# ranrhuang/SPFSplatV2

Hardware: AMD Instinct MI355X
Metric: Mpixels/s fwd+bwd, 256x256 @ ~65k Gaussians (higher is better)
Workload: dtype f32; 1 GPU; C2: 65536 pixel-aligned Gaussians/scene, 1 SH coefficient(s) per channel (sh_degree 0), 256x256, 8 scenes x 4 views per GPU per step, decoder fwd + MSE + bwd to all Gaussian parameters and poses; loss=spfsplatv2_amd.mse_loss (fused HIP), scenes_per_gpu=8, sh_coeffs=1, pair_buffer=planned from step 0 (x1.25 = 2814155 pairs), verified on device, launch=hip-graph replay, api=batched: one decoder call for all renders

## Files before the change

### spfsplatv2_amd/csrc/binning.hip

```cpp
#include <atomic>

#include "spf_common.h"
#include "launchers.h"

namespace spf {

uint32_t dense_threshold();
uint32_t dense_threshold_fwd();

constexpr int kScanThreads = 1024;

__global__ __launch_bounds__(kScanThreads) void spf_tile_scan_kernel(const uint32_t* __restrict__ count,
                                                                     uint32_t* __restrict__ start,
                                                                     uint32_t* __restrict__ fill,
                                                                     const uint32_t* __restrict__ flags,
                                                                     uint32_t dense_thr,
                                                                     uint32_t* __restrict__ counters, int n,
                                                                     const uint32_t* __restrict__ blk_total,
                                                                     uint32_t* __restrict__ blk_base, int nb) {
    constexpr int kWaves = kScanThreads / kWave;
    __shared__ uint32_t s_a[kWaves], s_b[kWaves], s_mx[kWaves], s_dn[kWaves];
    const int lane = threadIdx.x & (kWave - 1), wave = threadIdx.x >> 6;
    const int sega = ((n + kWaves - 1) / kWaves + kWave - 1) / kWave * kWave;
    const int segb = ((nb + kWaves - 1) / kWaves + kWave - 1) / kWave * kWave;
    const int a0 = min(n, wave * sega), a1 = min(n, a0 + sega), b0 = min(nb, wave * segb), b1 = min(nb, b0 + segb);
    uint32_t sa = 0, sb = 0, mx = 0, dn = 0;
    for (int i = a0 + lane; i < a1; i += kWave) {
        const uint32_t c = count[i];
        sa += c;
        mx = max(mx, c);
        dn += tile_is_dense(flags[i], c, dense_thr) ? 1u : 0u;
    }
    for (int i = b0 + lane; i < b1; i += kWave) sb += blk_total[i];
    sa = wave_sum_u32(sa); sb = wave_sum_u32(sb); mx = wave_max_u32(mx); dn = wave_sum_u32(dn);
    if (lane == 0) { s_a[wave] = sa; s_b[wave] = sb; s_mx[wave] = mx; s_dn[wave] = dn; }
    __syncthreads();
    uint32_t runa = 0, runb = 0, total = 0, gmax = 0, dense = 0;
#pragma unroll
    for (int w = 0; w < kWaves; ++w) {
        if (w < wave) { runa += s_a[w]; runb += s_b[w]; }
        total += s_a[w];
        gmax = max(gmax, s_mx[w]);
        dense += s_dn[w];
    }
    for (int i0 = a0; i0 < a1; i0 += kWave) {
        const int i = i0 + lane;
        const uint32_t c = i < a1 ? count[i] : 0u;
        const uint32_t inc = wave_iscan_u32(c);
        if (i < a1) { start[i] = runa + inc - c; fill[i] = 0u; }
        runa += (uint32_t)__builtin_amdgcn_readlane((int)inc, kWave - 1);
    }
    for (int i0 = b0; i0 < b1; i0 += kWave) {
        const int i = i0 + lane;
        const uint32_t c = i < b1 ? blk_total[i] : 0u;
        const uint32_t inc = wave_iscan_u32(c);
        if (i < b1) blk_base[i] = runb + inc - c;
        runb += (uint32_t)__builtin_amdgcn_readlane((int)inc, kWave - 1);
    }
    if (threadIdx.x == 0) {
        start[n] = total;
        counters[0] = total;
        counters[1] = gmax;
        counters[2] = 0;
        counters[3] = dense;
    }
}

__global__ __launch_bounds__(kScanThreads) void spf_tile_scan_render_kernel(const uint32_t* __restrict__ count,
                                                                            uint32_t* __restrict__ start,
                                                                            const uint32_t* __restrict__ flags,
                                                                            uint32_t dense_thr,
                                                                            uint32_t* __restrict__ counters, int T,
                                                                            const uint32_t* __restrict__ blk_total,
                                                                            uint32_t* __restrict__ blk_base, int nb) {
    constexpr int kWaves = kScanThreads / kWave;
    __shared__ uint32_t s_red[kWaves], s_a[kWaves], s_b[kWaves], s_mx[kWaves], s_dn[kWaves];
    const int r = blockIdx.x, R = gridDim.x;
    const int lane = threadIdx.x & (kWave - 1), wave = threadIdx.x >> 6;
    uint32_t pre = 0;
    for (int i = threadIdx.x; i < r * T; i += kScanThreads) pre += count[i];
    pre = wave_sum_u32(pre);
    if (lane == 0) s_red[wave] = pre;
    count += (size_t)r * T; flags += (size_t)r * T; start += (size_t)r * T;
    blk_total += (size_t)r * nb; blk_base += (size_t)r * nb;
    const int sega = ((T + kWaves - 1) / kWaves + kWave - 1) / kWave * kWave;
    const int segb = ((nb + kWaves - 1) / kWaves + kWave - 1) / kWave * kWave;
    const int a0 = min(T, wave * sega), a1 = min(T, a0 + sega), b0 = min(nb, wave * segb), b1 = min(nb, b0 + segb);
    uint32_t sa = 0, sb = 0, mx = 0, dn = 0;
    for (int i = a0 + lane; i < a1; i += kWave) {
        const uint32_t c = count[i];
        sa += c;
        mx = max(mx, c);
        dn += tile_is_dense(flags[i], c, dense_thr) ? 1u : 0u;
    }
    for (int i = b0 + lane; i < b1; i += kWave) sb += blk_total[i];
    sa = wave_sum_u32(sa); sb = wave_sum_u32(sb); mx = wave_max_u32(mx); dn = wave_sum_u32(dn);
    if (lane == 0) { s_a[wave] = sa; s_b[wave] = sb; s_mx[wave] = mx; s_dn[wave] = dn; }
    __syncthreads();
    uint32_t base = 0, runa = 0, runb = 0, total = 0, gmax = 0, dense = 0;
#pragma unroll
    for (int w = 0; w < kWaves; ++w) {
        base += s_red[w];
        if (w < wave) { runa += s_a[w]; runb += s_b[w]; }
        total += s_a[w];
        gmax = max(gmax, s_mx[w]);
        dense += s_dn[w];
    }
    runa += base; runb += base;
    for (int i0 = a0; i0 < a1; i0 += kWave) {
        const int i = i0 + lane;
        const uint32_t c = i < a1 ? count[i] : 0u;
        const uint32_t inc = wave_iscan_u32(c);
        if (i < a1) start[i] = runa + inc - c;
        runa += (uint32_t)__builtin_amdgcn_readlane((int)inc, kWave - 1);
    }
    for (int i0 = b0; i0 < b1; i0 += kWave) {
        const int i = i0 + lane;
        const uint32_t c = i < b1 ? blk_total[i] : 0u;
        const uint32_t inc = wave_iscan_u32(c);
        if (i < b1) blk_base[i] = runb + inc - c;
        runb += (uint32_t)__builtin_amdgcn_readlane((int)inc, kWave - 1);
    }
    if (threadIdx.x == 0) {
        if (gmax) atomicMax(&counters[1], gmax);
        if (dense) atomicAdd(&counters[3], dense);
        if (r == R - 1) {
            start[T] = base + total;
            counters[0] = base + total;
        }
    }
}

__global__ __launch_bounds__(kBlock) void spf_bin_pairs_kernel(const float* __restrict__ zkey,
                                                               const uint32_t* __restrict__ rect,
                                                               const uint32_t* __restrict__ tile_start,
                                                               uint32_t* __restrict__ tile_fill,
                                                               uint32_t* __restrict__ counters,
                                                               uint64_t* __restrict__ pairs, uint64_t capacity,
                                                               const uint32_t* __restrict__ blk_base,
                                                               uint32_t* __restrict__ pair_off,
                                                               int G, int T, int tiles_x, int lds,
                                                               uint32_t max_tile_hint) {
    extern __shared__ __attribute__((aligned(16))) uint32_t s_bin[];
    __shared__ uint32_t s_wtot[4];
    uint32_t* s_cnt = s_bin;
    uint32_t* s_base = s_bin + T;
    const int r = blockIdx.y;
    const int g = blockIdx.x * kBlock + threadIdx.x;
    if (r == 0 && g == 0) {
        uint32_t flag = counters[0] > capacity ? 1u : 0u;
        if (max_tile_hint != 0u && counters[1] > max_tile_hint) flag |= 2u;
        if (flag) counters[2] = flag;
    }
    if (counters[0] > capacity) return;
    const bool live = g < G;
    const size_t rg = (size_t)r * G + (live ? g : 0);
    const size_t tb = (size_t)r * T;
    const uint32_t rc = live ? rect[rg] : 0u;
    const float zk = live ? zkey[rg] : 0.f;
    const uint32_t bbase = blk_base[(size_t)r * gridDim.x + blockIdx.x];
    constexpr int kPre = 4;
    uint32_t ts_pre[kPre] = {0u, 0u, 0u, 0u};
    const bool pre = lds && T <= kPre * kBlock;
    if (pre) {
#pragma unroll
        for (int k = 0; k < kPre; ++k)
            if (threadIdx.x + k * kBlock < T) ts_pre[k] = tile_start[tb + threadIdx.x + k * kBlock];
    }
    const int x0 = rc & 0xff, y0 = (rc >> 8) & 0xff, x1 = (rc >> 16) & 0xff, y1 = rc >> 24;
    const bool any = x1 > x0 && y1 > y0;
    const int lane = threadIdx.x & 63, wave = threadIdx.x >> 6;
    const uint32_t cnt = any ? (uint32_t)((x1 - x0) * (y1 - y0)) : 0u;
    const uint32_t inc = wave_iscan_u32(cnt);
    if (lane == kWave - 1) s_wtot[wave] = inc;
    if (lds)
        for (int t = threadIdx.x; t < T; t += kBlock) s_cnt[t] = 0;
    __syncthreads();
    {
        uint32_t off = bbase + inc - cnt;
        for (int w = 0; w < wave; ++w) off += s_wtot[w];
        if (live) reinterpret_cast<uint2*>(pair_off)[rg] = make_uint2(rc, off);
    }
    const uint64_t key = any ? (((uint64_t)__float_as_uint(zk) << 32) | (uint32_t)g) : 0ull;
    if (!lds) {
        if (any)
            for (int ty = y0; ty < y1; ++ty)
                for (int tx = x0; tx < x1; ++tx) {
                    const size_t t = tb + ty * tiles_x + tx;
                    pairs[tile_start[t] + atomicAdd(&tile_fill[t], 1u)] = key;
                }
        return;
    }
    const bool single = any && cnt == 1u;
    const int stile = single ? y0 * tiles_x + x0 : -1;
    const LaneRun run = lane_runs(stile, lane);
    const bool run_head = single && run.head == lane;
    if (run_head) atomicAdd(&s_cnt[stile], (uint32_t)run.len);
    if (any && !single)
        for (int ty = y0; ty < y1; ++ty)
            for (int tx = x0; tx < x1; ++tx) atomicAdd(&s_cnt[ty * tiles_x + tx], 1u);
    __syncthreads();
    if (pre) {
#pragma unroll
        for (int k = 0; k < kPre; ++k) {
            const int t = threadIdx.x + k * kBlock;
            if (t < T) {
                const uint32_t c = s_cnt[t];
                if (c) {
                    s_base[t] = ts_pre[k] + atomicAdd(&tile_fill[tb + t], c);
                    s_cnt[t] = 0;
                }
            }
        }
    } else {
        for (int t = threadIdx.x; t < T; t += kBlock) {
            const uint32_t c = s_cnt[t];
            if (c) {
                s_base[t] = tile_start[tb + t] + atomicAdd(&tile_fill[tb + t], c);
                s_cnt[t] = 0;
            }
        }
    }
    __syncthreads();
    uint32_t first = 0u;
    if (run_head) first = atomicAdd(&s_cnt[stile], (uint32_t)run.len);
    first = (uint32_t)__shfl((int)first, run.head, kWave);
    if (single) pairs[s_base[stile] + first + (uint32_t)(lane - run.head)] = key;
    if (any && !single)
        for (int ty = y0; ty < y1; ++ty)
            for (int tx = x0; tx < x1; ++tx) {
                const int t = ty * tiles_x + tx;
                pairs[s_base[t] + atomicAdd(&s_cnt[t], 1u)] = key;
            }
}

template <int VB>
__global__ __launch_bounds__(kBlock) void spf_bin_pairs_views_kernel(const float* __restrict__ zkey,
                                                                     const uint32_t* __restrict__ rect,
                                                                     const uint32_t* __restrict__ tile_start,
                                                                     uint32_t* __restrict__ tile_fill,
                                                                     uint32_t* __restrict__ counters,
                                                                     uint64_t* __restrict__ pairs, uint64_t capacity,
                                                                     const uint32_t* __restrict__ blk_base,
                                                                     uint32_t* __restrict__ pair_off,
                                                                     int G, int T, int tiles_x, int V, int nvb,
                                                                     uint32_t max_tile_hint) {
    extern __shared__ __attribute__((aligned(16))) uint32_t s_bin[];
    __shared__ uint32_t s_wtot[VB][4];
    uint32_t* const s_cnt = s_bin;
    uint32_t* const s_base = s_bin + VB * T;
    const int sc = blockIdx.y / nvb, vb = blockIdx.y - sc * nvb;
    const int v0 = vb * VB, nv = min(VB, V - v0);
    const int r0 = sc * V + v0;
    const int g = blockIdx.x * kBlock + threadIdx.x;
    if (blockIdx.y == 0 && g == 0) {
        uint32_t flag = counters[0] > capacity ? 1u : 0u;
        if (max_tile_hint != 0u && counters[1] > max_tile_hint) flag |= 2u;
        if (flag) counters[2] = flag;
    }
    if (counters[0] > capacity) return;
    const bool live = g < G;
    const int lane = threadIdx.x & 63, wave = threadIdx.x >> 6;
    constexpr int kPre = 4;
    uint32_t rc[VB], bbase[VB], ts_pre[VB][kPre];
    float zk[VB];
#pragma unroll
    for (int k = 0; k < VB; ++k) {
        const bool on = k < nv;
        const size_t rg = (size_t)(r0 + (on ? k : 0)) * G + (live ? g : 0);
        rc[k] = (on && live) ? rect[rg] : 0u;
        zk[k] = (on && live) ? zkey[rg] : 0.f;
        bbase[k] = on ? blk_base[(size_t)(r0 + k) * gridDim.x + blockIdx.x] : 0u;
#pragma unroll
        for (int j = 0; j < kPre; ++j) {
            const int t = threadIdx.x + j * kBlock;
            ts_pre[k][j] = (on && t < T) ? tile_start[(size_t)(r0 + k) * T + t] : 0u;
        }
    }
    uint32_t cnt[VB], inc[VB];
#pragma unroll
    for (int k = 0; k < VB; ++k) {
        const int x0 = rc[k] & 0xff, y0 = (rc[k] >> 8) & 0xff, x1 = (rc[k] >> 16) & 0xff, y1 = rc[k] >> 24;
        cnt[k] = (x1 > x0 && y1 > y0) ? (uint32_t)((x1 - x0) * (y1 - y0)) : 0u;
        inc[k] = wave_iscan_u32(cnt[k]);
        if (lane == kWave - 1) s_wtot[k][wave] = inc[k];
    }
    for (int t = threadIdx.x; t < VB * T; t += kBlock) s_cnt[t] = 0;
    __syncthreads();
#pragma unroll
    for (int k = 0; k < VB; ++k) {
        uint32_t off = bbase[k] + inc[k] - cnt[k];
        for (int w = 0; w < wave; ++w) off += s_wtot[k][w];
        if (live && k < nv) reinterpret_cast<uint2*>(pair_off)[(size_t)(r0 + k) * G + g] = make_uint2(rc[k], off);
    }
    LaneRun run[VB];
    int stile[VB];
#pragma unroll
    for (int k = 0; k < VB; ++k) {
        const int x0 = rc[k] & 0xff, y0 = (rc[k] >> 8) & 0xff, x1 = (rc[k] >> 16) & 0xff, y1 = rc[k] >> 24;
        stile[k] = cnt[k] == 1u ? y0 * tiles_x + x0 : -1;
        run[k] = lane_runs(stile[k], lane);
        uint32_t* __restrict__ c = s_cnt + k * T;
        if (cnt[k] == 1u && run[k].head == lane) atomicAdd(&c[stile[k]], (uint32_t)run[k].len);
        if (cnt[k] > 1u)
            for (int ty = y0; ty < y1; ++ty)
                for (int tx = x0; tx < x1; ++tx) atomicAdd(&c[ty * tiles_x + tx], 1u);
    }
    __syncthreads();
#pragma unroll
    for (int k = 0; k < VB; ++k)
#pragma unroll
        for (int j = 0; j < kPre; ++j) {
            const int t = threadIdx.x + j * kBlock;
            if (k < nv && t < T) {
                const uint32_t c = s_cnt[k * T + t];
                if (c) {
                    s_base[k * T + t] = ts_pre[k][j] + atomicAdd(&tile_fill[(size_t)(r0 + k) * T + t], c);
                    s_cnt[k * T + t] = 0;
                }
            }
        }
    __syncthreads();
#pragma unroll
    for (int k = 0; k < VB; ++k) {
        const int x0 = rc[k] & 0xff, y0 = (rc[k] >> 8) & 0xff, x1 = (rc[k] >> 16) & 0xff, y1 = rc[k] >> 24;
        const uint64_t key = ((uint64_t)__float_as_uint(zk[k]) << 32) | (uint32_t)g;
        uint32_t* __restrict__ c = s_cnt + k * T;
        const uint32_t* __restrict__ bs = s_base + k * T;
        const bool single = cnt[k] == 1u;
        uint32_t first = 0u;
        if (single && run[k].head == lane) first = atomicAdd(&c[stile[k]], (uint32_t)run[k].len);
        first = (uint32_t)__shfl((int)first, run[k].head, kWave);
        if (single) pairs[bs[stile[k]] + first + (uint32_t)(lane - run[k].head)] = key;
        if (cnt[k] > 1u)
            for (int ty = y0; ty < y1; ++ty)
                for (int tx = x0; tx < x1; ++tx) {
                    const int t = ty * tiles_x + tx;
                    pairs[bs[t] + atomicAdd(&c[t], 1u)] = key;
                }
    }
}

constexpr int kOrderClasses = 64;
constexpr int kOrderWindow = 256;
static_assert(kOrderClasses == kWave, "the class bases are one wave's prefix sum");
__host__ __device__ inline int order_windows(int RT) { return ((RT >> 3) + kOrderWindow - 1) / kOrderWindow; }
__device__ __forceinline__ void tile_order_block(int id, const uint32_t* __restrict__ count,
                                                 const uint32_t* __restrict__ flags, uint2* __restrict__ order, int RT,
                                                 int T, uint32_t cap, uint32_t dense_thr, uint32_t dense_thr_fwd) {
    auto dense_bits = [&](uint32_t f, uint32_t n) {
        return (tile_is_dense(f, n, dense_thr) ? kOrderDenseBwd : 0u) | (tile_is_dense(f, n, dense_thr_fwd) ? kOrderDenseFwd : 0u);
    };
    __shared__ uint32_t s_cnt[kOrderClasses];
    const int nwin = order_windows(RT), x = id / nwin, w = id - x * nwin;
    const XcdMap xm = xcd_map(RT, T);
    const int per = RT >> 3, j0 = w * kOrderWindow, lo = x * per + j0, len = min(kOrderWindow, per - j0);
    const int nthr = (int)blockDim.x;
    if (w + 1 < nwin) {
        for (int i = threadIdx.x; i < len; i += nthr) {
            const int vid = xcd_tile(xm, T, x, j0 + i);
            const uint32_t n = min(count[vid], cap);
            order[lo + i] = make_uint2((uint32_t)vid | dense_bits(flags[vid], n), n);
        }
        return;
    }
    if (threadIdx.x < kOrderClasses) s_cnt[threadIdx.x] = 0u;
    __syncthreads();
    auto cls = [&](uint32_t n) {
        return (uint32_t)(kOrderClasses - 1) - min((uint32_t)(kOrderClasses - 1), n * (uint32_t)kOrderClasses / (cap + 1u));
    };
    for (int i = threadIdx.x; i < len; i += nthr) atomicAdd(&s_cnt[cls(min(count[xcd_tile(xm, T, x, j0 + i)], cap))], 1u);
    __syncthreads();
    uint32_t base = 0u;
    if (threadIdx.x < kWave) {
        const uint32_t c = s_cnt[threadIdx.x];
        base = wave_iscan_u32(c) - c;
    }
    __syncthreads();
    if (threadIdx.x < kWave) s_cnt[threadIdx.x] = base;
    __syncthreads();
    for (int i = threadIdx.x; i < len; i += nthr) {
        const int vid = xcd_tile(xm, T, x, j0 + i);
        const uint32_t n = min(count[vid], cap);
        const uint32_t pos = atomicAdd(&s_cnt[cls(n)], 1u);
        order[lo + pos] = make_uint2((uint32_t)vid | dense_bits(flags[vid], n), n);
    }
}
__global__ __launch_bounds__(kBlock) void spf_tile_order_kernel(const uint32_t* __restrict__ count,
                                                                const uint32_t* __restrict__ flags,
                                                                uint2* __restrict__ order, int RT, int T, uint32_t cap,
                                                                uint32_t dense_thr, uint32_t dense_thr_fwd) {
    tile_order_block((int)blockIdx.x, count, flags, order, RT, T, cap, dense_thr, dense_thr_fwd);
}

template <int THREADS>
__global__ __launch_bounds__(THREADS) void spf_sort_tiles_lds_kernel(TileLists tl,
                                                                     const uint32_t* __restrict__ counters,
                                                                     uint64_t* __restrict__ pairs,
                                                                     uint64_t capacity, uint32_t lo, uint32_t hi) {
    extern __shared__ __attribute__((aligned(16))) unsigned char smem_raw[];
    uint64_t* s = reinterpret_cast<uint64_t*>(smem_raw);
    if (counters[0] > capacity) return;
    uint32_t b, n;
    tile_range(tl, blockIdx.x, b, n);
    if (n <= lo || n > hi) return;
    uint64_t* __restrict__ p = pairs + b;
    for (uint32_t i = threadIdx.x; i < n; i += THREADS) s[i] = p[i];
    __syncthreads();
    uint32_t m = 1;
    while (m < n) m <<= 1;
    const uint32_t half = m >> 1;
    for (uint32_t k = 2; k <= m; k <<= 1) {
        for (uint32_t j = k >> 1; j > 0; j >>= 1) {
            const uint32_t mask = (j == (k >> 1)) ? (k - 1) : j;
            for (uint32_t i = threadIdx.x; i < half; i += THREADS) {
                const uint32_t a = ((i & ~(j - 1)) << 1) | (i & (j - 1));
                const uint32_t c = a ^ mask;
                if (c < n) {
                    const uint64_t x = s[a], y = s[c];
                    if (x > y) { s[a] = y; s[c] = x; }
                }
            }
            __syncthreads();
        }
    }
    for (uint32_t i = threadIdx.x; i < n; i += THREADS) p[i] = s[i];
}

__device__ __forceinline__ void cswap_u64(uint64_t& a, uint64_t& b) {
    const bool sw = a > b;
    const uint64_t lo = sw ? b : a, hi = sw ? a : b;
    a = lo;
    b = hi;
}

template <int CTRL>
__device__ __forceinline__ uint32_t dpp_mov_u32(uint32_t v) {
    return (uint32_t)__builtin_amdgcn_update_dpp((int)v, (int)v, CTRL, 0xf, 0xf, true);
}
template <int MASK>
__device__ __forceinline__ uint32_t lane_xor_u32(uint32_t v) {
    if constexpr (MASK == 1) return dpp_mov_u32<0xB1>(v);
    else if constexpr (MASK == 2) return dpp_mov_u32<0x4E>(v);
    else if constexpr (MASK == 3) return dpp_mov_u32<0x1B>(v);
    else if constexpr (MASK == 4) return dpp_mov_u32<0x1B>(dpp_mov_u32<0x141>(v));
    else if constexpr (MASK == 7) return dpp_mov_u32<0x141>(v);
    else if constexpr (MASK == 8) return dpp_mov_u32<0x128>(v);
    else if constexpr (MASK == 15) return dpp_mov_u32<0x140>(v);
    else return (uint32_t)__shfl_xor((int)v, MASK, kWave);
}
template <int MASK>
__device__ __forceinline__ uint64_t lane_xor_u64(uint64_t v) {
    return ((uint64_t)lane_xor_u32<MASK>((uint32_t)(v >> 32)) << 32) | lane_xor_u32<MASK>((uint32_t)v);
}

template <int E, int J>
__device__ __forceinline__ void thread_steps_down(uint64_t (&r)[E]) {
    if constexpr (J >= 1) {
#pragma unroll
        for (int s = 0; s < E; ++s)
            if (s < (s ^ J)) cswap_u64(r[s], r[s ^ J]);
        thread_steps_down<E, J / 2>(r);
    }
}
template <int E, int K>
__device__ __forceinline__ void merges_inside(uint64_t (&r)[E]) {
    if constexpr (K <= E) {
#pragma unroll
        for (int s = 0; s < E; ++s)
            if (s < (s ^ (K - 1))) cswap_u64(r[s], r[s ^ (K - 1)]);
        thread_steps_down<E, K / 4>(r);
        merges_inside<E, 2 * K>(r);
    }
}
template <int E, int MASK, bool MIRROR>
__device__ __forceinline__ void lane_step(uint64_t (&r)[E], int lane) {
    const bool lower = (lane & (MIRROR ? (MASK + 1) >> 1 : MASK)) == 0;
    uint64_t o[E];
#pragma unroll
    for (int s = 0; s < E; ++s) o[s] = lane_xor_u64<MASK>(r[MIRROR ? E - 1 - s : s]);
#pragma unroll
    for (int s = 0; s < E; ++s) r[s] = ((o[s] < r[s]) == lower) ? o[s] : r[s];
}
template <int E, int J>
__device__ __forceinline__ void lane_steps_down(uint64_t (&r)[E], int lane) {
    if constexpr (J >= E) {
        lane_step<E, J / E, false>(r, lane);
        lane_steps_down<E, J / 2>(r, lane);
    }
}
template <int E, int K>
__device__ __forceinline__ void merges_across(uint64_t (&r)[E], int lane) {
    if constexpr (K <= kWave * E) {
        lane_step<E, K / E - 1, true>(r, lane);
        lane_steps_down<E, K / 4>(r, lane);
        thread_steps_down<E, E / 2>(r);
        merges_across<E, 2 * K>(r, lane);
    }
}

template <int E>
__device__ __forceinline__ void sort_tile_in_wave(uint64_t* __restrict__ p, uint32_t n) {
    const int lane = threadIdx.x & (kWave - 1);
    uint64_t r[E];
#pragma unroll
    for (int s = 0; s < E; ++s) {
        const uint32_t e = (uint32_t)(E * lane + s);
        r[s] = e < n ? p[e] : ~0ull;
    }
    merges_inside<E, 2>(r);
    merges_across<E, 2 * E>(r, lane);
#pragma unroll
    for (int s = 0; s < E; ++s) {
        const uint32_t e = (uint32_t)(E * lane + s);
        if (e < n) p[e] = r[s];
    }
}

template <int E, bool SMALL>
__global__ __launch_bounds__(kBlock) void spf_sort_tiles_wave_kernel(TileLists tl, const uint32_t* __restrict__ flags,
                                                                     uint32_t* __restrict__ counters,
                                                                     uint64_t* __restrict__ pairs, uint64_t capacity,
                                                                     uint32_t lo, int RT,
                                                                     uint32_t dense_thr, uint2* __restrict__ order, int T, uint32_t dense_thr_fwd) {
    if (counters[0] > capacity) return;
    const int ob = order ? 8 * order_windows(RT) : 0;
    if ((int)blockIdx.x < ob) {
        tile_order_block((int)blockIdx.x, tl.count, flags, order, RT, T, tl.cap, dense_thr, dense_thr_fwd);
        return;
    }
    const int tile = ((int)blockIdx.x - ob) * (kBlock / kWave) + (threadIdx.x >> 6);
    if (tile >= RT) return;
    uint32_t b, n;
    tile_range(tl, tile, b, n);
    if (n <= lo || n > (uint32_t)(kWave * E)) return;
    if (SMALL) {
        if (n <= 2u * kWave) sort_tile_in_wave<2>(pairs + b, n);
        else if (n <= 4u * kWave) sort_tile_in_wave<4>(pairs + b, n);
        else if (E <= 8 || n <= 8u * kWave) sort_tile_in_wave<8>(pairs + b, n);
        else sort_tile_in_wave<16>(pairs + b, n);
    } else {
        sort_tile_in_wave<E>(pairs + b, n);
    }
}

template <int E, bool MIRROR>
__device__ __forceinline__ void block_step(uint64_t (&r)[E], uint64_t* __restrict__ s, int t, int tmask) {
#pragma unroll
    for (int k = 0; k < E; ++k) s[k * kBlock + t] = r[k];
    __syncthreads();
    const int pt = t ^ tmask;
    const bool lower = (t & (MIRROR ? (tmask + 1) >> 1 : tmask)) == 0;
#pragma unroll
    for (int k = 0; k < E; ++k) {
        const uint64_t o = s[(MIRROR ? E - 1 - k : k) * kBlock + pt];
        r[k] = ((o < r[k]) == lower) ? o : r[k];
    }
    __syncthreads();
}

template <int E>
__device__ __forceinline__ void sort_tile_in_block(uint64_t* __restrict__ p, uint32_t n, uint64_t* __restrict__ s_x) {
    const int t = threadIdx.x, lane = t & (kWave - 1);
    uint64_t r[E];
#pragma unroll
    for (int k = 0; k < E; ++k) {
        const uint32_t e = (uint32_t)(E * t + k);
        r[k] = e < n ? p[e] : ~0ull;
    }
    merges_inside<E, 2>(r);
    merges_across<E, 2 * E>(r, lane);
    block_step<E, true>(r, s_x, t, 127);
    lane_steps_down<E, 32 * E>(r, lane);
    thread_steps_down<E, E / 2>(r);
    block_step<E, true>(r, s_x, t, 255);
    block_step<E, false>(r, s_x, t, 64);
    lane_steps_down<E, 32 * E>(r, lane);
    thread_steps_down<E, E / 2>(r);
#pragma unroll
    for (int k = 0; k < E; ++k) {
        const uint32_t e = (uint32_t)(E * t + k);
        if (e < n) p[e] = r[k];
    }
}

template <int E>
__global__ __launch_bounds__(kBlock) void spf_sort_tiles_block_kernel(TileLists tl,
                                                                      const uint32_t* __restrict__ counters,
                                                                      uint64_t* __restrict__ pairs, uint64_t capacity,
                                                                      uint32_t lo) {
    __shared__ uint64_t s_x[E * kBlock];
    if (counters[0] > capacity) return;
    uint32_t b, n;
    tile_range(tl, blockIdx.x, b, n);
    if (n <= lo || n > (uint32_t)(kBlock * E)) return;
    sort_tile_in_block<E>(pairs + b, n, s_x);
}

template <int E, bool MIRROR>
__device__ __forceinline__ void pair_step(uint64_t (&r)[E], uint64_t* __restrict__ s, int t, int tmask) {
    constexpr int NT = 2 * kWave;
#pragma unroll
    for (int k = 0; k < E; ++k) s[k * NT + t] = r[k];
    __syncthreads();
    const int pt = t ^ tmask;
    const bool lower = (t & (MIRROR ? (tmask + 1) >> 1 : tmask)) == 0;
#pragma unroll
    for (int k = 0; k < E; ++k) {
        const uint64_t o = s[(MIRROR ? E - 1 - k : k) * NT + pt];
        r[k] = ((o < r[k]) == lower) ? o : r[k];
    }
}
template <int E>
__device__ __forceinline__ void sort_tile_in_pair(uint64_t* __restrict__ p, uint32_t n, uint64_t* __restrict__ s_x) {
    const int t = threadIdx.x, lane = t & (kWave - 1);
    uint64_t r[E];
#pragma unroll
    for (int k = 0; k < E; ++k) {
        const uint32_t e = (uint32_t)(E * t + k);
        r[k] = e < n ? p[e] : ~0ull;
    }
    merges_inside<E, 2>(r);
    merges_across<E, 2 * E>(r, lane);
    pair_step<E, true>(r, s_x, t, 127);
    lane_steps_down<E, 32 * E>(r, lane);
    thread_steps_down<E, E / 2>(r);
#pragma unroll
    for (int k = 0; k < E; ++k) {
        const uint32_t e = (uint32_t)(E * t + k);
        if (e < n) p[e] = r[k];
    }
}
__global__ __launch_bounds__(2 * kWave) void spf_sort_tiles_pair_kernel(TileLists tl, const uint32_t* __restrict__ flags,
                                                                        uint32_t* __restrict__ counters,
                                                                        uint64_t* __restrict__ pairs, uint64_t capacity,
                                                                        int RT, uint32_t dense_thr,
                                                                        uint2* __restrict__ order, int T, uint32_t dense_thr_fwd) {
    __shared__ uint64_t s_x[8 * 2 * kWave];
    if (counters[0] > capacity) return;
    const int ob = order ? 8 * order_windows(RT) : 0;
    if ((int)blockIdx.x < ob) {
        tile_order_block((int)blockIdx.x, tl.count, flags, order, RT, T, tl.cap, dense_thr, dense_thr_fwd);
        return;
    }
    const int tile = (int)blockIdx.x - ob;
    uint32_t b, n;
    tile_range(tl, tile, b, n);
    if (n <= 1u || n > 1024u) return;
    if (n <= 4u * kWave) {
        if (threadIdx.x >= kWave) return;
        if (n <= 2u * kWave) sort_tile_in_wave<2>(pairs + b, n);
        else sort_tile_in_wave<4>(pairs + b, n);
        return;
    }
    if (n <= 8u * kWave) sort_tile_in_pair<4>(pairs + b, n, s_x);
    else sort_tile_in_pair<8>(pairs + b, n, s_x);
}

template <bool BIG>
__global__ __launch_bounds__(kBlock) void spf_sort_tiles_mixed_kernel(TileLists tl, const uint32_t* __restrict__ flags,
                                                                      uint32_t* __restrict__ counters,
                                                                      uint64_t* __restrict__ pairs, uint64_t capacity,
                                                                      int RT, uint32_t dense_thr,
                                                                      uint2* __restrict__ order, int T, uint32_t dense_thr_fwd) {
    __shared__ uint64_t s_x[(BIG ? 16 : 8) * kBlock];
    if (counters[0] > capacity) return;
    const int ob = order ? 8 * order_windows(RT) : 0;
    if ((int)blockIdx.x < ob) {
        tile_order_block((int)blockIdx.x, tl.count, flags, order, RT, T, tl.cap, dense_thr, dense_thr_fwd);
        return;
    }
    int blk = (int)blockIdx.x - ob;
    if (BIG) {
        if (blk < RT) {
            uint32_t b, n;
            tile_range(tl, blk, b, n);
            if (n > 2048u && n <= 4096u) sort_tile_in_block<16>(pairs + b, n, s_x);
            return;
        }
        blk -= RT;
    }
    if (blk < RT) {
        uint32_t b, n;
        tile_range(tl, blk, b, n);
        if (n <= 512u || n > 2048u) return;
        if (n <= 1024u) sort_tile_in_block<4>(pairs + b, n, s_x);
        else sort_tile_in_block<8>(pairs + b, n, s_x);
        return;
    }
    const int tile = (blk - RT) * (kBlock / kWave) + (threadIdx.x >> 6);
    if (tile >= RT) return;
    uint32_t b, n;
    tile_range(tl, tile, b, n);
    if (n <= 1u || n > 512u) return;
    if (n <= 2u * kWave) sort_tile_in_wave<2>(pairs + b, n);
    else if (n <= 4u * kWave) sort_tile_in_wave<4>(pairs + b, n);
    else sort_tile_in_wave<8>(pairs + b, n);
}

constexpr uint32_t kBigChunk = 16384;

__device__ __forceinline__ void lds_steps(uint64_t* s, uint32_t cn, uint32_t kfirst, uint32_t klast) {
    const uint32_t half = kBigChunk >> 1;
    for (uint32_t k = kfirst; k <= klast; k <<= 1) {
        for (uint32_t j = k >> 1; j > 0; j >>= 1) {
            const uint32_t mask = (j == (k >> 1)) ? (k - 1) : j;
            for (uint32_t i = threadIdx.x; i < half; i += 1024) {
                const uint32_t a = ((i & ~(j - 1)) << 1) | (i & (j - 1));
                const uint32_t c = a ^ mask;
                if (c < cn) {
                    const uint64_t x = s[a], y = s[c];
                    if (x > y) { s[a] = y; s[c] = x; }
                }
            }
            __syncthreads();
        }
    }
}
__device__ __forceinline__ void lds_tail(uint64_t* s, uint32_t cn) {
    const uint32_t half = kBigChunk >> 1;
    for (uint32_t j = kBigChunk >> 1; j > 0; j >>= 1) {
        for (uint32_t i = threadIdx.x; i < half; i += 1024) {
            const uint32_t a = ((i & ~(j - 1)) << 1) | (i & (j - 1));
            const uint32_t c = a ^ j;
            if (c < cn) {
                const uint64_t x = s[a], y = s[c];
                if (x > y) { s[a] = y; s[c] = x; }
            }
        }
        __syncthreads();
    }
}

__global__ __launch_bounds__(1024) void spf_sort_tiles_big_kernel(TileLists tl,
                                                                  const uint32_t* __restrict__ counters,
                                                                  uint64_t* pairs, uint64_t capacity, uint32_t lo) {
    extern __shared__ __attribute__((aligned(16))) unsigned char smem_raw[];
    uint64_t* s = reinterpret_cast<uint64_t*>(smem_raw);
    if (counters[0] > capacity) return;
    uint32_t b, n;
    tile_range(tl, blockIdx.x, b, n);
    if (n <= lo) return;
    uint64_t* p = pairs + b;
    uint32_t m = 1;
    while (m < n) m <<= 1;
    for (uint32_t c0 = 0; c0 < n; c0 += kBigChunk) {
        const uint32_t cn = min(kBigChunk, n - c0);
        for (uint32_t i = threadIdx.x; i < cn; i += 1024) s[i] = p[c0 + i];
        __syncthreads();
        lds_steps(s, cn, 2, kBigChunk);
        for (uint32_t i = threadIdx.x; i < cn; i += 1024) p[c0 + i] = s[i];
        __syncthreads();
    }
    for (uint32_t k = 2 * kBigChunk; k <= m; k <<= 1) {
        for (uint32_t j = k >> 1; j >= kBigChunk; j >>= 1) {
            const uint32_t mask = (j == (k >> 1)) ? (k - 1) : j;
            for (uint32_t i = threadIdx.x; i < (m >> 1); i += 1024) {
                const uint32_t a = ((i & ~(j - 1)) << 1) | (i & (j - 1));
                const uint32_t c = a ^ mask;
                if (c < n) {
                    const uint64_t x = p[a], y = p[c];
                    if (x > y) { p[a] = y; p[c] = x; }
                }
            }
            __threadfence_block();
            __syncthreads();
        }
        for (uint32_t c0 = 0; c0 < n; c0 += kBigChunk) {
            const uint32_t cn = min(kBigChunk, n - c0);
            for (uint32_t i = threadIdx.x; i < cn; i += 1024) s[i] = p[c0 + i];
            __syncthreads();
            lds_tail(s, cn);
            for (uint32_t i = threadIdx.x; i < cn; i += 1024) p[c0 + i] = s[i];
            __syncthreads();
        }
    }
}

hipError_t launch_tile_scan(const SpfState& st, int R, int T, int nblk, uint32_t dense_thr, bool zeroed,
                            hipStream_t stream) {
    if (zeroed && R > 1 && R <= 256 && (long)R * T <= (1L << 18))
        spf_tile_scan_render_kernel<<<R, kScanThreads, 0, stream>>>(st.tile_count, st.tile_start, st.tile_flags,
                                                                    dense_thr, st.counters, T, st.blk_total,
                                                                    st.blk_base, nblk);
    else
        spf_tile_scan_kernel<<<1, kScanThreads, 0, stream>>>(st.tile_count, st.tile_start, st.tile_fill, st.tile_flags,
                                                             dense_thr, st.counters, R * T, st.blk_total, st.blk_base,
                                                             R * nblk);
    return hipGetLastError();
}

hipError_t launch_bin_pairs(const SpfDims& d, const SpfState& st, uint64_t capacity, int T, int tiles_x,
                            uint32_t max_tile_hint, hipStream_t stream) {
    dim3 grid((d.G + kBlock - 1) / kBlock, d.S * d.V);
    const int lds = T <= max_lds_tiles() ? 1 : 0;
    const char* const want_env = getenv("SPF_BIN_VIEWS");
    const int want_vb = want_env ? atoi(want_env) : 0;
    const int nblk = (d.G + kBlock - 1) / kBlock;
    const int vb = want_vb ? (want_vb >= 2 ? 2 : 1) : (nblk >= 1024 ? 2 : 1);
    if (lds && vb == 2 && d.V >= 2 && T <= 4 * kBlock) {
        const int nvb = (d.V + 1) / 2;
        dim3 vgrid(nblk, d.S * nvb);
        spf_bin_pairs_views_kernel<2><<<vgrid, kBlock, (size_t)4 * T * sizeof(uint32_t), stream>>>(
            st.zkey, st.rect, st.tile_start, st.tile_fill, st.counters, st.pairs, capacity, st.blk_base, st.pair_off,
            d.G, T, tiles_x, d.V, nvb, max_tile_hint);
        return hipGetLastError();
    }
    spf_bin_pairs_kernel<<<grid, kBlock, lds ? 2 * sizeof(uint32_t) * T : 0, stream>>>(
        st.zkey, st.rect, st.tile_start, st.tile_fill, st.counters, st.pairs, capacity, st.blk_base, st.pair_off,
        d.G, T, tiles_x, lds, max_tile_hint);
    return hipGetLastError();
}

SortSwitches read_sort_switches() {
    const char* const b = getenv("SPF_SORT_BLOCKS");
    const char* const bm = getenv("SPF_SORT_BIG_MIXED");
    return {b ? b[0] == '1' : -1, getenv("SPF_SORT_SEPARATE") != nullptr, getenv("SPF_SORT_SINGLE") != nullptr,
            getenv("SPF_SORT_LDS_2K") != nullptr, !(bm && bm[0] == '0')};
}

int plan_tile_sort(uint32_t max_tile_hint, int tiles_call, bool with_order, const SortSwitches& sw, SortLaunch* out) {
    const uint32_t mx = max_tile_hint ? max_tile_hint : 0xffffffffu;
    const bool blocks = sw.blocks < 0 ? tiles_call < 6144 : sw.blocks == 1;
    int n = 0;
    uint32_t done = 1;
    const auto add = [&](int kernel, uint32_t hi) {
        out[n] = {kernel, done, hi, with_order && n == 0};
        ++n, done = hi;
    };
    if (with_order && mx <= 1) add(SPF_SORT_ORDER_ONLY, 1);
    while (done < mx) {
        if (done == 1 && blocks) {
            if (mx <= 512 || sw.separate) add(SPF_SORT_WAVE8, 512);
            else if (mx > 2048 && sw.big_mixed && !sw.lds_2k) add(SPF_SORT_MIXED_BIG, 4096);
            else add(SPF_SORT_MIXED, 2048);
        } else if (done == 1) {
            if (mx <= 1024 && !sw.single) add(SPF_SORT_PAIR, 1024);
            else if (mx <= 512) add(SPF_SORT_WAVE8, 512);
            else add(SPF_SORT_WAVE16, 1024);
        } else if (done == 512) add(SPF_SORT_BLOCK4, 1024);
        else if (done == 1024) add(blocks ? SPF_SORT_BLOCK8 : SPF_SORT_WAVE32, 2048);
        else if (done == 2048) sw.lds_2k ? add(SPF_SORT_LDS, 8192) : add(SPF_SORT_BLOCK16, 4096);
        else if (done <= 8192) add(SPF_SORT_LDS, 2 * done);
        else add(SPF_SORT_BIG, 0xffffffffu);
    }
    return n;
}

hipError_t launch_tile_sort(const SpfState& st, const TileLists& tl, int RT, int RT_call, uint64_t capacity,
                            uint32_t max_tile_hint, const uint2* order_c, int T,
                            hipStream_t stream) {
    uint2* order = const_cast<uint2*>(order_c);
    const uint32_t thr = dense_threshold(), thr_f = dense_threshold_fwd();
    const int wgrid = (RT + kBlock / kWave - 1) / (kBlock / kWave);
    SortLaunch plan[SPF_SORT_MAX_LAUNCHES];
    const int n = plan_tile_sort(max_tile_hint, RT_call, order != nullptr, read_sort_switches(), plan);
    for (const SortLaunch* l = plan; l < plan + n; ++l) {
        const int ob = l->order ? 8 * order_windows(RT) : 0;
        switch (l->kernel) {
        case SPF_SORT_ORDER_ONLY:
            spf_tile_order_kernel<<<ob, kBlock, 0, stream>>>(tl.count, st.tile_flags, order, RT, T, tl.cap, thr, thr_f);
            break;
        case SPF_SORT_MIXED_BIG:
            spf_sort_tiles_mixed_kernel<true><<<ob + 2 * RT + wgrid, kBlock, 0, stream>>>(
                tl, st.tile_flags, st.counters, st.pairs, capacity, RT, thr, order, T, thr_f);
            break;
        case SPF_SORT_MIXED:
            spf_sort_tiles_mixed_kernel<false><<<ob + RT + wgrid, kBlock, 0, stream>>>(
                tl, st.tile_flags, st.counters, st.pairs, capacity, RT, thr, order, T, thr_f);
            break;
        case SPF_SORT_PAIR:
            spf_sort_tiles_pair_kernel<<<ob + RT, 2 * kWave, 0, stream>>>(tl, st.tile_flags, st.counters, st.pairs, capacity,
                                                                          RT, thr, order, T, thr_f);
            break;
        case SPF_SORT_WAVE8:
            spf_sort_tiles_wave_kernel<8, true><<<ob + wgrid, kBlock, 0, stream>>>(
                tl, st.tile_flags, st.counters, st.pairs, capacity, l->lo, RT, thr, order, T, thr_f);
            break;
        case SPF_SORT_WAVE16:
            spf_sort_tiles_wave_kernel<16, true><<<ob + wgrid, kBlock, 0, stream>>>(
                tl, st.tile_flags, st.counters, st.pairs, capacity, l->lo, RT, thr, order, T, thr_f);
            break;
        case SPF_SORT_WAVE32:
            spf_sort_tiles_wave_kernel<32, false><<<wgrid, kBlock, 0, stream>>>(
                tl, st.tile_flags, st.counters, st.pairs, capacity, l->lo, RT, thr, nullptr, 0, thr_f);
            break;
        case SPF_SORT_BLOCK4:
            spf_sort_tiles_block_kernel<4><<<RT, kBlock, 0, stream>>>(tl, st.counters, st.pairs, capacity, l->lo);
            break;
        case SPF_SORT_BLOCK8:
            spf_sort_tiles_block_kernel<8><<<RT, kBlock, 0, stream>>>(tl, st.counters, st.pairs, capacity, l->lo);
            break;
        case SPF_SORT_BLOCK16:
            spf_sort_tiles_block_kernel<16><<<RT, kBlock, 0, stream>>>(tl, st.counters, st.pairs, capacity, l->lo);
            break;
        case SPF_SORT_LDS:
            if (l->hi > 8192) {
                static std::atomic<bool> attr_set[64];
                int dev = 0;
                if (hipGetDevice(&dev) != hipSuccess || dev < 0 || dev >= 64 || !attr_set[dev].load(std::memory_order_acquire)) {
                    hipError_t e = hipFuncSetAttribute(reinterpret_cast<const void*>(&spf_sort_tiles_lds_kernel<1024>),
                                                       hipFuncAttributeMaxDynamicSharedMemorySize, 16384 * 8);
                    if (e != hipSuccess) return e;
                    e = hipFuncSetAttribute(reinterpret_cast<const void*>(&spf_sort_tiles_big_kernel),
                                            hipFuncAttributeMaxDynamicSharedMemorySize, 16384 * 8);
                    if (e != hipSuccess) return e;
                    if (dev >= 0 && dev < 64) attr_set[dev].store(true, std::memory_order_release);
                }
            }
            spf_sort_tiles_lds_kernel<1024><<<RT, 1024, (size_t)l->hi * 8, stream>>>(tl, st.counters, st.pairs, capacity,
                                                                                     l->lo, l->hi);
            break;
        case SPF_SORT_BIG:
            spf_sort_tiles_big_kernel<<<RT, 1024, 16384 * 8, stream>>>(tl, st.counters, st.pairs, capacity, l->lo);
            break;
        }
    }
    return hipGetLastError();
}

}
```

Baseline: 5934 Mpixels/s.

## Sort tiles just above power-of-two sizes by splitting into head and tail runs

Tiles whose pair count is slightly above 256 or 512 are now sorted by bitonic-sorting a power-of-two head and a small tail run separately, then merging them with binary-search ranks. Previously such a tile was padded up to the next power-of-two bitonic network (512 or 1024 elements). The aim is to skip most of the padded compare-exchange work and barriers, at the cost of scattered global writes and per-key binary searches in LDS. The new path is on by default and can be turned off with SPF_SORT_SPLIT=0.

```diff
diff --git a/spfsplatv2_amd/csrc/binning.hip b/spfsplatv2_amd/csrc/binning.hip
--- a/spfsplatv2_amd/csrc/binning.hip
+++ b/spfsplatv2_amd/csrc/binning.hip
@@ -584,25 +584,32 @@
     }
 }
 
+constexpr uint32_t kSplitMax256 = 256 + 128, kSplitMax512 = 512 + 256;
+template <int HW, int NW>
+__device__ __forceinline__ void sort_tile_split(uint64_t* __restrict__ p, uint32_t n, uint64_t* __restrict__ s_x, int flip);
+
 template <int E>
 __global__ __launch_bounds__(kBlock) void spf_sort_tiles_block_kernel(TileLists tl,
                                                                       const uint32_t* __restrict__ counters,
                                                                       uint64_t* __restrict__ pairs, uint64_t capacity,
-                                                                      uint32_t lo) {
+                                                                      uint32_t lo, uint32_t split) {
     __shared__ uint64_t s_x[E * kBlock];
     if (counters[0] > capacity) return;
     uint32_t b, n;
     tile_range(tl, blockIdx.x, b, n);
     if (n <= lo || n > (uint32_t)(kBlock * E)) return;
-    sort_tile_in_block<E>(pairs + b, n, s_x);
-}
-
+    if (E == 4 && split && n > 512u && n <= kSplitMax512) sort_tile_split<2, 4>(pairs + b, n, s_x, 0);
+    else sort_tile_in_block<E>(pairs + b, n, s_x);
+}
+
+template <int E>
+__device__ __forceinline__ void pair_put(const uint64_t (&r)[E], uint64_t* __restrict__ s, int t) {
+#pragma unroll
+    for (int k = 0; k < E; ++k) s[k * 2 * kWave + t] = r[k];
+}
 template <int E, bool MIRROR>
-__device__ __forceinline__ void pair_step(uint64_t (&r)[E], uint64_t* __restrict__ s, int t, int tmask) {
+__device__ __forceinline__ void pair_get(uint64_t (&r)[E], const uint64_t* __restrict__ s, int t, int tmask) {
     constexpr int NT = 2 * kWave;
-#pragma unroll
-    for (int k = 0; k < E; ++k) s[k * NT + t] = r[k];
-    __syncthreads();
     const int pt = t ^ tmask;
     const bool lower = (t & (MIRROR ? (tmask + 1) >> 1 : tmask)) == 0;
 #pragma unroll
@@ -610,6 +617,12 @@
         const uint64_t o = s[(MIRROR ? E - 1 - k : k) * NT + pt];
         r[k] = ((o < r[k]) == lower) ? o : r[k];
     }
+}
+template <int E, bool MIRROR>
+__device__ __forceinline__ void pair_step(uint64_t (&r)[E], uint64_t* __restrict__ s, int t, int tmask) {
+    pair_put<E>(r, s, t);
+    __syncthreads();
+    pair_get<E, MIRROR>(r, s, t, tmask);
 }
 template <int E>
 __device__ __forceinline__ void sort_tile_in_pair(uint64_t* __restrict__ p, uint32_t n, uint64_t* __restrict__ s_x) {
@@ -631,11 +644,96 @@
         if (e < n) p[e] = r[k];
     }
 }
+template <int E>
+__device__ __forceinline__ void sort_run_in_wave(const uint64_t* __restrict__ p, uint32_t n, uint64_t* __restrict__ run,
+                                                 int lane) {
+    uint64_t r[E];
+#pragma unroll
+    for (int k = 0; k < E; ++k) {
+        const uint32_t e = (uint32_t)(E * lane + k);
+        r[k] = e < n ? p[e] : ~0ull;
+    }
+    merges_inside<E, 2>(r);
+    merges_across<E, 2 * E>(r, lane);
+#pragma unroll
+    for (int k = 0; k < E; ++k) run[E * lane + k] = r[k];
+}
+template <int K>
+__device__ __forceinline__ void ranks_in_run(const uint64_t* __restrict__ a, uint32_t N, const uint64_t (&key)[K],
+                                             uint32_t (&pos)[K]) {
+#pragma unroll
+    for (int k = 0; k < K; ++k) pos[k] = 0;
+    for (uint32_t s = N >> 1; s; s >>= 1) {
+#pragma unroll
+        for (int k = 0; k < K; ++k) pos[k] += a[pos[k] + s - 1] < key[k] ? s : 0u;
+    }
+#pragma unroll
+    for (int k = 0; k < K; ++k) pos[k] += a[pos[k]] < key[k] ? 1u : 0u;
+}
+template <int HW, int NW>
+__device__ __forceinline__ void sort_tile_split(uint64_t* __restrict__ p, uint32_t n, uint64_t* __restrict__ s_x, int flip) {
+    static_assert((HW == 1 && NW == 2) || (HW == 2 && (NW == 2 || NW == 4)), "head waves / waves of the block");
+    constexpr uint32_t Hd = 256u * HW;
+    const int t = threadIdx.x, lane = t & (kWave - 1), w = t >> 6;
+    const uint32_t m = n - Hd;
+    const uint32_t slots = m <= 64u ? 64u : m <= 128u ? 128u : 256u;
+    const bool head = HW == 1 ? w == flip : w < 2;
+    const int ht = HW == 1 ? lane : t;
+    const int tail_wave = HW == 1 ? 1 - flip : NW == 4 ? 2 : flip;
+    uint64_t r[4];
+    if (head) {
+#pragma unroll
+        for (int k = 0; k < 4; ++k) r[k] = p[4 * ht + k];
+        merges_inside<4, 2>(r);
+        merges_across<4, 8>(r, lane);
+    }
+    if (w == tail_wave) {
+        if (m <= 64u) sort_run_in_wave<1>(p + Hd, m, s_x + Hd, lane);
+        else if (HW == 1 || m <= 128u) sort_run_in_wave<2>(p + Hd, m, s_x + Hd, lane);
+        else sort_run_in_wave<4>(p + Hd, m, s_x + Hd, lane);
+    }
+    if (HW == 2) {
+        if (head) pair_put<4>(r, s_x, t);
+        __syncthreads();
+        if (head) {
+            pair_get<4, true>(r, s_x, t, 127);
+            lane_steps_down<4, 128>(r, lane);
+            thread_steps_down<4, 2>(r);
+        }
+        __syncthreads();
+    }
+    if (head) {
+#pragma unroll
+        for (int k = 0; k < 4; ++k) s_x[4 * ht + k] = r[k];
+    }
+    __syncthreads();
+    constexpr int NT = NW * kWave, HR = (int)Hd / NT, TR = ((int)Hd / 2 + NT - 1) / NT;
+    {
+        uint64_t key[HR];
+        uint32_t pos[HR];
+#pragma unroll
+        for (int k = 0; k < HR; ++k) key[k] = s_x[t + k * NT];
+        ranks_in_run<HR>(s_x + Hd, slots, key, pos);
+#pragma unroll
+        for (int k = 0; k < HR; ++k) p[(uint32_t)(t + k * NT) + pos[k]] = key[k];
+    }
+    {
+        uint64_t key[TR];
+        uint32_t pos[TR];
+#pragma unroll
+        for (int k = 0; k < TR; ++k) key[k] = (uint32_t)(t + k * NT) < m ? s_x[Hd + t + k * NT] : 0ull;
+        ranks_in_run<TR>(s_x, Hd, key, pos);
+#pragma unroll
+        for (int k = 0; k < TR; ++k)
+            if ((uint32_t)(t + k * NT) < m) p[(uint32_t)(t + k * NT) + pos[k]] = key[k];
+    }
+}
 __global__ __launch_bounds__(2 * kWave) void spf_sort_tiles_pair_kernel(TileLists tl, const uint32_t* __restrict__ flags,
                                                                         uint32_t* __restrict__ counters,
                                                                         uint64_t* __restrict__ pairs, uint64_t capacity,
                                                                         int RT, uint32_t dense_thr,
-                                                                        uint2* __restrict__ order, int T, uint32_t dense_thr_fwd) {
+                                                                        uint2* __restrict__ order, int T, uint32_t dense_thr_fwd,
+                                                                        uint32_t split) {
     __shared__ uint64_t s_x[8 * 2 * kWave];
     if (counters[0] > capacity) return;
     const int ob = order ? 8 * order_windows(RT) : 0;
@@ -653,7 +751,9 @@
         else sort_tile_in_wave<4>(pairs + b, n);
         return;
     }
-    if (n <= 8u * kWave) sort_tile_in_pair<4>(pairs + b, n, s_x);
+    if (split && n <= kSplitMax256) sort_tile_split<1, 2>(pairs + b, n, s_x, tile & 1);
+    else if (n <= 8u * kWave) sort_tile_in_pair<4>(pairs + b, n, s_x);
+    else if (split && n <= kSplitMax512) sort_tile_split<2, 2>(pairs + b, n, s_x, tile & 1);
     else sort_tile_in_pair<8>(pairs + b, n, s_x);
 }
 
@@ -662,7 +762,8 @@
                                                                       uint32_t* __restrict__ counters,
                                                                       uint64_t* __restrict__ pairs, uint64_t capacity,
                                                                       int RT, uint32_t dense_thr,
-                                                                      uint2* __restrict__ order, int T, uint32_t dense_thr_fwd) {
+                                                                      uint2* __restrict__ order, int T, uint32_t dense_thr_fwd,
+                                                                      uint32_t split) {
     __shared__ uint64_t s_x[(BIG ? 16 : 8) * kBlock];
     if (counters[0] > capacity) return;
     const int ob = order ? 8 * order_windows(RT) : 0;
@@ -684,7 +785,8 @@
         uint32_t b, n;
         tile_range(tl, blk, b, n);
         if (n <= 512u || n > 2048u) return;
-        if (n <= 1024u) sort_tile_in_block<4>(pairs + b, n, s_x);
+        if (split && n <= kSplitMax512) sort_tile_split<2, 4>(pairs + b, n, s_x, 0);
+        else if (n <= 1024u) sort_tile_in_block<4>(pairs + b, n, s_x);
         else sort_tile_in_block<8>(pairs + b, n, s_x);
         return;
     }
@@ -855,6 +957,8 @@
     const int wgrid = (RT + kBlock / kWave - 1) / (kBlock / kWave);
     SortLaunch plan[SPF_SORT_MAX_LAUNCHES];
     const int n = plan_tile_sort(max_tile_hint, RT_call, order != nullptr, read_sort_switches(), plan);
+    const char* const sp = getenv("SPF_SORT_SPLIT");
+    const uint32_t split = !(sp && sp[0] == '0');
     for (const SortLaunch* l = plan; l < plan + n; ++l) {
         const int ob = l->order ? 8 * order_windows(RT) : 0;
         switch (l->kernel) {
@@ -863,15 +967,15 @@
             break;
         case SPF_SORT_MIXED_BIG:
             spf_sort_tiles_mixed_kernel<true><<<ob + 2 * RT + wgrid, kBlock, 0, stream>>>(
-                tl, st.tile_flags, st.counters, st.pairs, capacity, RT, thr, order, T, thr_f);
+                tl, st.tile_flags, st.counters, st.pairs, capacity, RT, thr, order, T, thr_f, split);
             break;
         case SPF_SORT_MIXED:
             spf_sort_tiles_mixed_kernel<false><<<ob + RT + wgrid, kBlock, 0, stream>>>(
-                tl, st.tile_flags, st.counters, st.pairs, capacity, RT, thr, order, T, thr_f);
+                tl, st.tile_flags, st.counters, st.pairs, capacity, RT, thr, order, T, thr_f, split);
             break;
         case SPF_SORT_PAIR:
             spf_sort_tiles_pair_kernel<<<ob + RT, 2 * kWave, 0, stream>>>(tl, st.tile_flags, st.counters, st.pairs, capacity,
-                                                                          RT, thr, order, T, thr_f);
+                                                                          RT, thr, order, T, thr_f, split);
             break;
         case SPF_SORT_WAVE8:
             spf_sort_tiles_wave_kernel<8, true><<<ob + wgrid, kBlock, 0, stream>>>(
@@ -886,13 +990,13 @@
                 tl, st.tile_flags, st.counters, st.pairs, capacity, l->lo, RT, thr, nullptr, 0, thr_f);
             break;
         case SPF_SORT_BLOCK4:
-            spf_sort_tiles_block_kernel<4><<<RT, kBlock, 0, stream>>>(tl, st.counters, st.pairs, capacity, l->lo);
+            spf_sort_tiles_block_kernel<4><<<RT, kBlock, 0, stream>>>(tl, st.counters, st.pairs, capacity, l->lo, split);
             break;
         case SPF_SORT_BLOCK8:
-            spf_sort_tiles_block_kernel<8><<<RT, kBlock, 0, stream>>>(tl, st.counters, st.pairs, capacity, l->lo);
+            spf_sort_tiles_block_kernel<8><<<RT, kBlock, 0, stream>>>(tl, st.counters, st.pairs, capacity, l->lo, split);
             break;
         case SPF_SORT_BLOCK16:
-            spf_sort_tiles_block_kernel<16><<<RT, kBlock, 0, stream>>>(tl, st.counters, st.pairs, capacity, l->lo);
+            spf_sort_tiles_block_kernel<16><<<RT, kBlock, 0, stream>>>(tl, st.counters, st.pairs, capacity, l->lo, split);
             break;
         case SPF_SORT_LDS:
             if (l->hi > 8192) {
```

Result: no change. 5978 Mpixels/s, median of 6 (+0.8%).
